# hwwang55/GraphGAN

Measured on AMD Instinct MI355X. Metric: sampled_edges_per_sec, higher is better.
Workload: dtype f32

## Files before the change

### graphgan_amd/csrc/steps.hip

```cpp
#include <stdlib.h>

#include <algorithm>
#include <cmath>
#include <vector>

#include "gg_internal.h"

namespace gg {

struct HubAcc {
    unsigned long long *acc;
    int64_t cap;
    float scale;
};
__device__ __forceinline__ unsigned long long *hub_row(const HubAcc &h, int slot, int ld) {
    const int64_t k = -3 - (int64_t)slot;
    return (slot <= -3 && k < h.cap) ? h.acc + k * (ld + 1) : nullptr;
}
__device__ __forceinline__ void hub_add(unsigned long long *p, float x, float scale) {
    atomicAdd(p, (unsigned long long)__float2ll_rn(x * scale));
}

struct StepArgs {
    float *E, *b;
// ... 549 lines not shown
        }
        if (t == 0) {
            float var = a.b[row];
            const float g = a.gb[row];
            if (SGD) {
                var -= a.lr * g;
            } else {
                float m = a.mb[row], v = a.vb[row];
                adam_elem(var, m, v, g, a);
                a.mb[row] = m;
                a.vb[row] = v;
            }
            if (!__builtin_isfinite(var)) *a.bad = 1ull;
            a.b[row] = var;
            a.gb[row] = 0.f;
            a.touched[row] = 0;
            if (a.sg_cnt) a.sg_cnt[row] = 0;
        }
    }
}

constexpr int DET_MAX_PAIRS = 256;
constexpr int DET_THREADS = 1024;
constexpr int DET_GROUPS = DET_THREADS / 16;
constexpr size_t DET_LDS_ROW_BYTES = 144 * 1024;

__device__ __forceinline__ unsigned group16_ballot(bool pred) {
    const uint64_t m = __ballot(pred);
    return (unsigned)(m >> (threadIdx.x & 48)) & 0xffffu;
}

template <int NF, bool ROWS_IN_LDS, int OPT, bool SMALLN>
__global__ __launch_bounds__(DET_THREADS) void pair_grad_det_kernel(const StepArgs a, const OptArgs o) {
    static_assert(OPT == 0 || ROWS_IN_LDS, "the fused update needs every table read in front of the barrier");
    extern __shared__ float det_rows[];
    __shared__ int32_t ids[2 * DET_MAX_PAIRS];
    __shared__ float coef[DET_MAX_PAIRS], coefb[DET_MAX_PAIRS];
    const int t = threadIdx.x & 15, g = threadIdx.x >> 4;
    const int n = a.n, ld = a.ld, nchunk = ld >> 2;
    const float inv_n = a.n_glob ? 1.0f / (float)(*a.n_glob) : a.inv_n;
    const bool stamp = a.prof && blockIdx.x == 0 && (threadIdx.x == 0 || threadIdx.x == DET_THREADS - 64);
    unsigned long long *const pw = a.prof + (threadIdx.x ? 8 : 0);
    if (stamp) pw[0] = wall_clock64();
    for (int s = threadIdx.x; s < 2 * n; s += DET_THREADS) ids[s] = s < n ? a.u[s] : a.v[s - n];
    for (int p = g; p < n; p += DET_GROUPS) {
        const int iu = a.u[p], iv = a.v[p];
        const float xp = a.x[p];
        const float bv = a.b[iv];
        const float4 *ru = (const float4 *)(a.E + (int64_t)iu * ld);
        const float4 *rv = (const float4 *)(a.E + (int64_t)iv * ld);
        float acc = 0.f;
        for (int c = t; c < nchunk; c += 16) {
            const float4 x = ru[c], y = rv[c];
            if (ROWS_IN_LDS) {
                ((float4 *)(det_rows + (size_t)p * ld))[c] = x;
                ((float4 *)(det_rows + (size_t)(n + p) * ld))[c] = y;
            }
            acc = __builtin_fmaf(x.x, y.x, acc);
            acc = __builtin_fmaf(x.y, y.y, acc);
            acc = __builtin_fmaf(x.z, y.z, acc);
            acc = __builtin_fmaf(x.w, y.w, acc);
        }
        acc += __shfl_xor(acc, 8, 64);
        acc += __shfl_xor(acc, 4, 64);
        acc += __shfl_xor(acc, 2, 64);
        acc += __shfl_xor(acc, 1, 64);
        const float sc = acc + bv;
        const float sg = 1.0f / (1.0f + expf(-sc));
        float ds;
        if (a.is_d) {
            ds = sg - xp;
        } else {
            const bool inside = (sg >= 1e-5f) && (sg <= 1.0f);
            ds = inside ? -(xp * inv_n) * (1.0f - sg) : 0.0f;
        }
        if (t == 0) {
            coef[p] = ds;
            coefb[p] = a.is_d ? ds + a.lambda * bv : ds;
        }
    }
    if (stamp) pw[1] = wall_clock64();
    __syncthreads();
    if (stamp) pw[2] = wall_clock64();
    constexpr int NW = SMALLN ? 2 : 2 * DET_MAX_PAIRS / 64;
    constexpr int NFW = (NF + 3) / 4;
    constexpr int CB = 4;
    const int lane = threadIdx.x & 63;
    const int wave = __builtin_amdgcn_readfirstlane((int)(threadIdx.x >> 6));
    int idr[NW];
#pragma unroll
    for (int j = 0; j < NW; ++j) idr[j] = (64 * j + lane < 2 * n) ? ids[64 * j + lane] : -1;
    auto leader_of = [&](const int s, int &r, uint64_t (&m)[NW]) -> bool {
        r = __builtin_amdgcn_readlane(idr[0], s & 63);
#pragma unroll
        for (int j = 1; j < NW; ++j) r = (s >> 6) == j ? __builtin_amdgcn_readlane(idr[j], s & 63) : r;
        bool earlier = false;
#pragma unroll
        for (int j = 0; j < NW; ++j) {
            m[j] = __ballot(idr[j] == r);
            if (64 * j + 63 < s) earlier |= m[j] != 0ull;
            else if (64 * j <= s) earlier |= (m[j] & ((1ull << (s & 63)) - 1ull)) != 0ull;
        }
        return !earlier;
    };
    auto own_row = [&](const int s, const int r, const uint64_t (&m)[NW], const bool PRE, const float (&pm)[NFW], const float (&pv)[NFW], const float (&pb)[3]) {
        float own[NFW], lown[NFW], acc[NFW], accb = 0.f;
#pragma unroll
        for (int i = 0; i < NFW; ++i) {
            const int f = lane + 64 * i;
            own[i] = f < ld ? (ROWS_IN_LDS ? det_rows[(size_t)s * ld + f] : a.E[(int64_t)r * ld + f]) : 0.f;
            lown[i] = a.lambda * own[i];
            acc[i] = 0.f;
        }
#pragma unroll
        for (int j = 0; j < NW; ++j) {
            uint64_t cur = m[j];
            while (cur) {
                int sq[CB];
#pragma unroll
                for (int k = 0; k < CB; ++k) {
                    if (cur) { sq[k] = 64 * j + __builtin_ctzll(cur); cur &= cur - 1ull; }
                    else sq[k] = -1;
                }
                float c[CB], cb[CB], pr[CB][NFW];
#pragma unroll
                for (int k = 0; k < CB; ++k) {
                    const int sk = sq[k] >= 0 ? sq[k] : s;
                    const int p = sk < n ? sk : sk - n;
                    const int ps = sk < n ? n + p : p;
                    c[k] = coef[p];
                    cb[k] = coefb[p];
                    const float *prow = ROWS_IN_LDS ? det_rows + (size_t)ps * ld : a.E + (int64_t)ids[ps] * ld;
#pragma unroll
                    for (int i = 0; i < NFW; ++i) {
                        const int f = lane + 64 * i;
                        pr[k][i] = f < ld ? prow[f] : 0.f;
                    }
                }
#pragma unroll
                for (int k = 0; k < CB; ++k) {
                    if (sq[k] >= 0) {
#pragma unroll
                        for (int i = 0; i < NFW; ++i) acc[i] += c[k] * pr[k][i] + lown[i];
                        if (sq[k] >= n) accb += cb[k];
                    }
                }
            }
        }
        if (OPT == 0) {
            float *gr = a.gE + (int64_t)r * ld;
#pragma unroll
            for (int i = 0; i < NFW; ++i) {
                const int f = lane + 64 * i;
                if (f < ld) gr[f] = acc[i];
            }
            if (lane == 0) {
                a.gb[r] = accb;
                if (a.track) a.touched[r] = 1;
            }
        } else {
            const int64_t ro = (int64_t)r * ld;
#pragma unroll
            for (int i = 0; i < NFW; ++i) {
                const int f = lane + 64 * i;
                if (f < ld) {
                    float var = own[i];
                    if (OPT == 2) {
                        var -= o.lr * acc[i];
                    } else {
                        float m1 = PRE ? pm[i] : o.mE[ro + f], v1 = PRE ? pv[i] : o.vE[ro + f];
                        adam_elem(var, m1, v1, acc[i], o);
                        o.mE[ro + f] = m1;
                        o.vE[ro + f] = v1;
                    }
                    if (!__builtin_isfinite(var)) *o.bad = 1ull;
                    o.E[ro + f] = var;
                }
            }
            if (lane == 0) {
                float var = PRE ? pb[0] : o.b[r];
                if (OPT == 2) {
                    var -= o.lr * accb;
                } else {
                    float m1 = PRE ? pb[1] : o.mb[r], v1 = PRE ? pb[2] : o.vb[r];
                    adam_elem(var, m1, v1, accb, o);
                    o.mb[r] = m1;
                    o.vb[r] = v1;
                }
                if (!__builtin_isfinite(var)) *o.bad = 1ull;
                o.b[r] = var;
            }
        }
    };
    if constexpr (OPT != 0 && SMALLN && NFW <= 2) {
        constexpr int SPW = 2 * 64 / (DET_THREADS / 64);
        constexpr int SPH = SPW / 2;
#pragma clang loop unroll(full)
        for (int h0 = 0; h0 < SPW; h0 += SPH) {
            float pm[SPH][NFW], pv[SPH][NFW], pb[SPH][3];
#pragma clang loop unroll(full)
            for (int k = 0; k < SPH; ++k) {
                const int s = wave + (h0 + k) * (DET_THREADS / 64);
                int r = 0;
                uint64_t m[NW];
#pragma unroll
                for (int i = 0; i < NFW; ++i) { pm[k][i] = 0.f; pv[k][i] = 0.f; }
                pb[k][0] = pb[k][1] = pb[k][2] = 0.f;
                if (s < 2 * n && leader_of(s, r, m)) {
                    const int64_t ro = (int64_t)r * ld;
#pragma unroll
                    for (int i = 0; i < NFW; ++i) {
                        const int f = lane + 64 * i;
                        if (OPT == 1 && f < ld) { pm[k][i] = o.mE[ro + f]; pv[k][i] = o.vE[ro + f]; }
                    }
                    if (lane == 0) {
                        pb[k][0] = o.b[r];
                        if (OPT == 1) { pb[k][1] = o.mb[r]; pb[k][2] = o.vb[r]; }
                    }
                }
            }
#pragma clang loop unroll(full)
            for (int k = 0; k < SPH; ++k) {
                const int s = wave + (h0 + k) * (DET_THREADS / 64);
                int r = 0;
                uint64_t m[NW];
                if (s < 2 * n && leader_of(s, r, m)) own_row(s, r, m, true, pm[k], pv[k], pb[k]);
            }
        }
    } else {
        const float none[NFW] = {}, none3[3] = {};
        for (int s = (int)blockIdx.x * (DET_THREADS / 64) + wave; s < 2 * n; s += (int)gridDim.x * (DET_THREADS / 64)) {
            int r = 0;
            uint64_t m[NW];
            if (leader_of(s, r, m)) own_row(s, r, m, false, none, none, none3);
        }
    }
    if (stamp) pw[3] = wall_clock64();
}

static unsigned det_workgroups(int n) {
    static const int cap = [] { const char *e = getenv("GG_DET_WORKGROUPS"); return e ? std::max(1, atoi(e)) : 8; }();
    return (unsigned)std::min(cap, std::max(1, (2 * n + DET_THREADS / 64 - 1) / (DET_THREADS / 64)));
}

static bool det_lds_granted(int device);
static bool det_rows_fit_lds(const gg_ctx *ctx, const StepArgs &s) {
    return (size_t)2 * s.n * s.ld * sizeof(float) <= DET_LDS_ROW_BYTES && det_lds_granted(ctx->device);
}

template <int NF, int OPT>
static hipError_t launch_pair_grad_det_lds(gg_ctx *ctx, const StepArgs &s, const OptArgs &o) {
    static bool raised_dev[64] = {};
    bool &raised = raised_dev[ctx->device & 63];
    if (!raised) {
        hipError_t e = hipFuncSetAttribute((const void *)pair_grad_det_kernel<NF, true, OPT, true>, hipFuncAttributeMaxDynamicSharedMemorySize, (int)DET_LDS_ROW_BYTES);
        if (e == hipSuccess) e = hipFuncSetAttribute((const void *)pair_grad_det_kernel<NF, true, OPT, false>, hipFuncAttributeMaxDynamicSharedMemorySize, (int)DET_LDS_ROW_BYTES);
        if (e != hipSuccess) return e;
        raised = true;
    }
    const size_t dyn = (size_t)2 * s.n * s.ld * sizeof(float);
    const dim3 grid(OPT == 0 ? det_workgroups(s.n) : 1);
    if (s.n <= 64) hipLaunchKernelGGL((pair_grad_det_kernel<NF, true, OPT, true>), grid, dim3(DET_THREADS), dyn, ctx->stream, s, o);
    else hipLaunchKernelGGL((pair_grad_det_kernel<NF, true, OPT, false>), grid, dim3(DET_THREADS), dyn, ctx->stream, s, o);
    return hipSuccess;
}

static bool det_lds_granted(int device) {
    static int state[64] = {};
    int &s = state[device & 63];
    if (s == 0) {
        const hipError_t e = hipFuncSetAttribute((const void *)pair_grad_det_kernel<4, true, 0, true>, hipFuncAttributeMaxDynamicSharedMemorySize, (int)DET_LDS_ROW_BYTES);
        if (e != hipSuccess) (void)hipGetLastError();
        s = e == hipSuccess ? 1 : -1;
    }
    return s > 0;
}

template <int NF>
static hipError_t launch_pair_grad_det(gg_ctx *ctx, const StepArgs &s, const OptArgs &o, int opt) {
    if (!det_rows_fit_lds(ctx, s)) {
        const dim3 grid(det_workgroups(s.n));
        if (s.n <= 64) hipLaunchKernelGGL((pair_grad_det_kernel<NF, false, 0, true>), grid, dim3(DET_THREADS), 0, ctx->stream, s, o);
        else hipLaunchKernelGGL((pair_grad_det_kernel<NF, false, 0, false>), grid, dim3(DET_THREADS), 0, ctx->stream, s, o);
        return hipSuccess;
    }
    if (opt == 1) return launch_pair_grad_det_lds<NF, 1>(ctx, s, o);
    if (opt == 2) return launch_pair_grad_det_lds<NF, 2>(ctx, s, o);
    return launch_pair_grad_det_lds<NF, 0>(ctx, s, o);
}

template <int SGD>
__global__ __launch_bounds__(256) void sparse_opt_kernel(const OptArgs a) {
    const int t = threadIdx.x & 15;
    const int g0 = (blockIdx.x * blockDim.x + threadIdx.x) >> 4;
    const int ng = (gridDim.x * blockDim.x) >> 4;
    const int cnt = (int)*a.touched_total;
    const int nchunk = a.ld >> 2;
    for (int r = g0; r < cnt; r += ng) opt_row<SGD>(a, a.touched_list[r], t, nchunk);
}

constexpr int STAGE_SORT = 64;

template <int MODE>
__global__ __launch_bounds__(256) void staged_opt_kernel(const OptArgs a) {
    constexpr bool SGD = MODE == 1;
    __shared__ int32_t perm_s[16][STAGE_SORT];
    const int t = threadIdx.x & 15;
    int32_t *const perm = perm_s[threadIdx.x >> 4];
    const int64_t g0 = ((int64_t)blockIdx.x * blockDim.x + threadIdx.x) >> 4, ng = ((int64_t)gridDim.x * blockDim.x) >> 4;
    const int64_t n_rows = a.sg_tot[0];
    const int nchunk = a.ld >> 2;
    for (int64_t r = g0; r < n_rows; r += ng) {
        const int4 e = a.sg_list[r];
        const int row = e.x, n = e.z;
        const float4 *const seg = (const float4 *)(a.stage + (int64_t)e.y * a.ld);
        const float *const sb = a.stage_b + e.y;
        const int32_t *const key = a.stage_key + e.y;
        float4 g[4];
#pragma unroll
        for (int i = 0; i < 4; ++i) g[i] = make_float4(0.f, 0.f, 0.f, 0.f);
        float gbias = 0.f;
        auto add_row = [&](const float4 *src) {
#pragma unroll
            for (int i = 0; i < 4; ++i) {
                const int c = t + 16 * i;
                if (c < nchunk) {
                    const float4 x = src[c];
                    g[i].x += x.x; g[i].y += x.y; g[i].z += x.z; g[i].w += x.w;
                }
            }
        };
        if (n <= STAGE_SORT) {
            if (n > 1) {
                int k[4], rk[4];
#pragma unroll
                for (int i = 0; i < 4; ++i) {
                    k[i] = (t + 16 * i < n) ? key[t + 16 * i] : 0x7fffffff;
                    rk[i] = 0;
                }
#pragma unroll
                for (int j = 0; j < 4; ++j) {
                    if (16 * j < n) {
                        const int nl = min(n - 16 * j, 16);
                        for (int l = 0; l < nl; ++l) {
                            const int kk = __shfl(k[j], l, 16);
#pragma unroll
                            for (int i = 0; i < 4; ++i) rk[i] += kk < k[i];
                        }
                    }
                }
#pragma unroll
                for (int i = 0; i < 4; ++i)
                    if (t + 16 * i < n) perm[rk[i]] = t + 16 * i;
            } else if (t == 0) {
                perm[0] = 0;
            }
            __builtin_amdgcn_fence(__ATOMIC_RELEASE, "wavefront");
            __builtin_amdgcn_wave_barrier();
            __builtin_amdgcn_fence(__ATOMIC_ACQUIRE, "wavefront");
            int o = 0;
            for (; o + 4 <= n; o += 4) {
                const float4 *s0 = seg + (int64_t)perm[o] * nchunk, *s1 = seg + (int64_t)perm[o + 1] * nchunk;
                const float4 *s2 = seg + (int64_t)perm[o + 2] * nchunk, *s3 = seg + (int64_t)perm[o + 3] * nchunk;
#pragma unroll
                for (int i = 0; i < 4; ++i) {
                    const int c = t + 16 * i;
                    if (c < nchunk) {
                        const float4 x0 = s0[c], x1 = s1[c], x2 = s2[c], x3 = s3[c];
                        g[i].x += x0.x; g[i].y += x0.y; g[i].z += x0.z; g[i].w += x0.w;
                        g[i].x += x1.x; g[i].y += x1.y; g[i].z += x1.z; g[i].w += x1.w;
                        g[i].x += x2.x; g[i].y += x2.y; g[i].z += x2.z; g[i].w += x2.w;
                        g[i].x += x3.x; g[i].y += x3.y; g[i].z += x3.z; g[i].w += x3.w;
                    }
                }
            }
            for (; o < n; ++o) add_row(seg + (int64_t)perm[o] * nchunk);
            for (int q = t; q < n; q += 16) gbias += sb[perm[q]];
            __builtin_amdgcn_wave_barrier();
        } else {
            int last = -1;
            for (int q = 0; q < n; ++q) {
                int best = 0x7fffffff, besto = 0;
                for (int o = t; o < n; o += 16) {
                    const int kk = key[o];
                    if (kk > last && kk < best) { best = kk; besto = o; }
                }
#pragma unroll
                for (int m = 8; m >= 1; m >>= 1) {
                    const int ob = __shfl_xor(best, m, 16), oo = __shfl_xor(besto, m, 16);
                    if (ob < best) { best = ob; besto = oo; }
                }
                add_row(seg + (int64_t)besto * nchunk);
                if ((q & 15) == t) gbias += sb[besto];
                last = best;
            }
        }
        gbias += __shfl_xor(gbias, 8, 64);
        gbias += __shfl_xor(gbias, 4, 64);
        gbias += __shfl_xor(gbias, 2, 64);
        gbias += __shfl_xor(gbias, 1, 64);
        const int64_t o4 = ((int64_t)row * a.ld) >> 2;
        if (MODE == 2) {
#pragma unroll
            for (int i = 0; i < 4; ++i) {
                const int c = t + 16 * i;
                if (c < nchunk) ((float4 *)a.gE)[o4 + c] = g[i];
            }
            if (t == 0) {
                a.gb[row] = gbias;
                a.touched[row] = 1;
                a.sg_cnt[row] = 0;
            }
            continue;
        }
#pragma unroll
        for (int i = 0; i < 4; ++i) {
            const int c = t + 16 * i;
            if (c >= nchunk) continue;
            float4 var = ((float4 *)a.E)[o4 + c];
            if (SGD) {
                var.x -= a.lr * g[i].x; var.y -= a.lr * g[i].y; var.z -= a.lr * g[i].z; var.w -= a.lr * g[i].w;
            } else {
                float4 m = ((float4 *)a.mE)[o4 + c], v = ((float4 *)a.vE)[o4 + c];
                adam_elem(var.x, m.x, v.x, g[i].x, a);
                adam_elem(var.y, m.y, v.y, g[i].y, a);
                adam_elem(var.z, m.z, v.z, g[i].z, a);
                adam_elem(var.w, m.w, v.w, g[i].w, a);
                ((float4 *)a.mE)[o4 + c] = m;
                ((float4 *)a.vE)[o4 + c] = v;
            }
            if (nonfinite4(var)) *a.bad = 1ull;
            ((float4 *)a.E)[o4 + c] = var;
        }
        if (t == 0) {
            float var = a.b[row];
            if (SGD) {
                var -= a.lr * gbias;
            } else {
                float m = a.mb[row], v = a.vb[row];
                adam_elem(var, m, v, gbias, a);
                a.mb[row] = m;
                a.vb[row] = v;
            }
            if (!__builtin_isfinite(var)) *a.bad = 1ull;
            a.b[row] = var;
            a.sg_cnt[row] = 0;
        }
    }
}

__global__ void add_word_kernel(int64_t *dst, const int64_t *src) { *dst += *src; }

__global__ __launch_bounds__(256) void pack_rows_kernel(float *gE, float *gb, int32_t *touched, const int32_t *list, const int64_t *cnt_ptr,
                                                        int64_t cap, int ld, int32_t *out_ids, float *out_rows, int32_t *err) {
    const int t = threadIdx.x & 15;
    const int64_t g0 = ((int64_t)blockIdx.x * blockDim.x + threadIdx.x) >> 4, ng = ((int64_t)gridDim.x * blockDim.x) >> 4;
    const int64_t cnt = *cnt_ptr;
    if (cnt > cap && blockIdx.x == 0 && threadIdx.x == 0) *err = 1;
    for (int64_t r = g0; r < cap; r += ng) {
        if (r >= cnt) {
            if (t == 0) out_ids[r] = -1;
            continue;
        }
        const int row = list[r];
        float *src = gE + (int64_t)row * ld, *dst = out_rows + r * (ld + 1);
        for (int f = t; f < ld; f += 16) { dst[f] = src[f]; src[f] = 0.f; }
        if (t == 0) { dst[ld] = gb[row]; gb[row] = 0.f; out_ids[r] = row; touched[row] = 0; }
    }
}

__device__ __forceinline__ uint16_t f32_to_bf16(float x) {
    uint32_t u = __builtin_bit_cast(uint32_t, x);
    if ((u & 0x7fffffffu) > 0x7f800000u) return (uint16_t)((u >> 16) | 0x40u);
    u += 0x7fffu + ((u >> 16) & 1u);
    return (uint16_t)(u >> 16);
}
__device__ __forceinline__ float bf16_to_f32(uint16_t h) { return __builtin_bit_cast(float, (uint32_t)h << 16); }
static inline size_t pack_row_words(int ld, bool bf16) { return bf16 ? (size_t)(ld + 2) / 2 : (size_t)ld + 1; }
template <bool BF16> __device__ __forceinline__ float pack_get(const float *rows, int64_t r, int ld, int f) {
    if (BF16) return bf16_to_f32(((const uint16_t *)rows)[r * (ld + 2) + f]);
    return rows[r * (ld + 1) + f];
}
template <bool BF16> __device__ __forceinline__ void pack_put(float *rows, int64_t r, int ld, int f, float v) {
    if (BF16) ((uint16_t *)rows)[r * (ld + 2) + f] = f32_to_bf16(v);
    else rows[r * (ld + 1) + f] = v;
}

template <bool BF16 = false>
__global__ __launch_bounds__(256) void add_rows_kernel(float *gE, float *gb, int32_t *touched, const int32_t *ids, const float *rows, int64_t cnt,
                                                       int ld) {
    const int t = threadIdx.x & 15;
    const int64_t g0 = ((int64_t)blockIdx.x * blockDim.x + threadIdx.x) >> 4, ng = ((int64_t)gridDim.x * blockDim.x) >> 4;
    for (int64_t r = g0; r < cnt; r += ng) {
        const int row = ids[r];
        if (row < 0) continue;
        float *dst = gE + (int64_t)row * ld;
        for (int f = t; f < ld; f += 16) dst[f] += pack_get<BF16>(rows, r, ld, f);
        if (t == 0) { gb[row] += pack_get<BF16>(rows, r, ld, ld); touched[row] = 1; }
    }
}


int apply_optimizer(gg_ctx *ctx, int which, int64_t n);
void step_done(gg_ctx *ctx, int which, int64_t n);
int run_path_step(gg_ctx *ctx);

static OptArgs make_opt_args(gg_ctx *ctx, int which) {
    Model &M = ctx->model[which];
    OptArgs o{};
    o.E = M.E; o.b = M.b; o.mE = M.mE; o.vE = M.vE; o.mb = M.mb; o.vb = M.vb; o.gE = ctx->gradE; o.gb = ctx->gradb;
    o.nE = (int64_t)ctx->n_node * ctx->ld;
    o.n_node = ctx->n_node; o.ld = ctx->ld;
    o.b1 = ctx->cfg.adam_beta1; o.b2 = ctx->cfg.adam_beta2; o.eps = ctx->cfg.adam_eps;
    o.lr = M.lr;
    o.lr_t = (M.lr * sqrtf(1.0f - M.b2p)) / (1.0f - M.b1p);
    o.touched = ctx->touched; o.touched_list = ctx->touched_list; o.touched_cnt = ctx->touched_cnt;
    o.bad = ctx->table_bad.as<unsigned long long>() + which;
    return o;
}

__global__ void set_count_kernel(int64_t *dst, int64_t v) { *dst = v; }

static int global_pair_count(gg_ctx *ctx, int64_t n_local, const int64_t **out) {
    *out = nullptr;
    const int world = ctx->comm ? ctx->world : ctx->fake_world;
    if (world <= 1) return GG_OK;
    GG_HIP(ctx, ctx->x_nglob.reserve(sizeof(int64_t) * 2));
    int64_t *w = ctx->x_nglob.as<int64_t>();
    hipLaunchKernelGGL(set_count_kernel, dim3(1), dim3(1), 0, ctx->stream, w, ctx->comm ? n_local : n_local * world);
    if (ctx->comm) {
        int rc = comm_allreduce_i64(ctx, w, 1);
        if (rc != GG_OK) return rc;
    }
    *out = w;
    return GG_OK;
}

static int64_t stage_bytes_cap() {
    static const int64_t cap = [] {
        const char *e = getenv("GG_STAGE_MAX_BYTES");
        return e ? (int64_t)atoll(e) : (int64_t)24 << 30;
    }();
    return cap;
}

__global__ __launch_bounds__(256) void hub_index_kernel(const int32_t *cnt, int64_t n, int T, int32_t *off, int32_t *rows, int64_t *nhub) {
    const int64_t i = (int64_t)blockIdx.x * blockDim.x + threadIdx.x;
    if (i >= n || cnt[i] <= T) return;
    const int h = (int)atomicAdd((unsigned long long *)nhub, 1ull);
    off[i] = h;
    rows[h] = (int32_t)i;
}

__global__ __launch_bounds__(256) void hub_finalize_kernel(unsigned long long *acc, const int32_t *rows, const int64_t *nhub, int64_t cap, int ld,
                                                           double inv_scale, float *gE, float *gb) {
    const int64_t n = min(*nhub, cap) * (ld + 1);
    for (int64_t i = (int64_t)blockIdx.x * blockDim.x + threadIdx.x; i < n; i += (int64_t)gridDim.x * blockDim.x) {
        const unsigned long long v = acc[i];
        if (!v) continue;
        acc[i] = 0ull;
        const int64_t h = i / (ld + 1);
        const int f = (int)(i - h * (ld + 1));
        const float x = (float)((double)(long long)v * inv_scale);
        if (f < ld) gE[(int64_t)rows[h] * ld + f] += x;
        else gb[rows[h]] += x;
    }
}

static float hub_scale(bool per_pair_mean, int64_t n) {
    return std::ldexp(1.0f, 32 + (per_pair_mean && n > 1 ? (int)std::ilogb((double)n) : 0));
}

static HubAcc hub_args(gg_ctx *ctx, float scale) {
    return HubAcc{ctx->hub_acc.as<unsigned long long>(), ctx->hub_cap, scale};
}

static int hub_index(gg_ctx *ctx, const int32_t *cnt, int32_t *off, DevBuf &rows, int64_t *tot, hipStream_t stream) {
    GG_HIP(ctx, rows.reserve(sizeof(int32_t) * (size_t)ctx->n_node));
    GG_HIP(ctx, hipMemsetAsync(tot + 2, 0, sizeof(int64_t), stream));
    hipLaunchKernelGGL(hub_index_kernel, dim3((unsigned)cdiv(ctx->n_node, 256)), dim3(256), 0, stream, cnt, (int64_t)ctx->n_node, ctx->sg_threshold, off,
                       rows.as<int32_t>(), tot + 2);
    GG_HIP(ctx, hipGetLastError());
    return GG_OK;
}

static void hub_finalize(gg_ctx *ctx, bool early_index, float scale, float *gE, float *gb) {
    DevBuf &rows = early_index ? ctx->sgp_hub : ctx->sg_hub, &tot = early_index ? ctx->sgp_tot : ctx->sg_tot;
    const int64_t n = ctx->hub_cap * (ctx->ld + 1);
    const unsigned nb = (unsigned)std::max<int64_t>(1, std::min<int64_t>(cdiv(n, 256), 2048));
    hipLaunchKernelGGL(hub_finalize_kernel, dim3(nb), dim3(256), 0, ctx->stream, ctx->hub_acc.as<unsigned long long>(), rows.as<int32_t>(),
                       tot.as<int64_t>() + 2, ctx->hub_cap, ctx->ld, 1.0 / (double)scale, gE, gb);
}

static int staged_reserve(gg_ctx *ctx, int64_t n_occ, int64_t n_stage) {
    if (n_stage * (int64_t)(ctx->ld + 2) * 4 > stage_bytes_cap()) return 1;
    const size_t cnt_before = ctx->sg_cnt.bytes;
    GG_HIP(ctx, ctx->sg_cnt.reserve(sizeof(int32_t) * (size_t)ctx->n_node));
    const bool was_dirty = ctx->sg_cnt_dirty;
    if (ctx->sg_cnt.bytes != cnt_before || ctx->sg_cnt_dirty) GG_HIP(ctx, hipMemsetAsync(ctx->sg_cnt.p, 0, ctx->sg_cnt.bytes, ctx->stream));
    ctx->sg_cnt_dirty = true;
    GG_HIP(ctx, ctx->sg_off.reserve(sizeof(int32_t) * (size_t)ctx->n_node));
    GG_HIP(ctx, ctx->sg_list.reserve(sizeof(int4) * (size_t)ctx->n_node));
    GG_HIP(ctx, ctx->sg_slot.reserve(sizeof(int32_t) * (size_t)n_occ));
    GG_HIP(ctx, ctx->sg_bias.reserve(sizeof(float) * (size_t)n_stage));
    GG_HIP(ctx, ctx->sg_key.reserve(sizeof(int32_t) * (size_t)n_stage));
    GG_HIP(ctx, ctx->sg_tot.reserve(sizeof(int64_t) * 4));
    {
        const int64_t cap = std::min<int64_t>(ctx->n_node, n_occ / ((int64_t)ctx->sg_threshold + 1) + 1);
        const size_t before = ctx->hub_acc.bytes;
        if (ctx->hub_acc.reserve(sizeof(unsigned long long) * (size_t)cap * (ctx->ld + 1)) != hipSuccess) {
            (void)hipGetLastError();
            ctx->hub_cap = 0;
            return 1;
        }
        if (ctx->hub_acc.bytes != before || was_dirty) GG_HIP(ctx, hipMemsetAsync(ctx->hub_acc.p, 0, ctx->hub_acc.bytes, ctx->stream));
        ctx->hub_cap = (int64_t)(ctx->hub_acc.bytes / (sizeof(unsigned long long) * (ctx->ld + 1)));
    }
    if (ctx->sg_rows.reserve(sizeof(float) * (size_t)n_stage * ctx->ld) != hipSuccess) {
        (void)hipGetLastError();
        return 1;
    }
    return GG_OK;
}

static int staged_finish(gg_ctx *ctx, int which, int64_t n, int64_t n_occ, bool early_index = false) {
    const int opt = ctx->cfg.optimizer;
    OptArgs o = make_opt_args(ctx, which);
    DevBuf &b_cnt = early_index ? ctx->sgp_cnt : ctx->sg_cnt, &b_list = early_index ? ctx->sgp_list : ctx->sg_list;
    DevBuf &b_tot = early_index ? ctx->sgp_tot : ctx->sg_tot, &b_key = early_index ? ctx->sgp_key : ctx->sg_key;
    o.sg_cnt = b_cnt.as<int32_t>(); o.sg_list = b_list.as<int4>(); o.sg_tot = b_tot.as<int64_t>();
    o.stage = ctx->sg_rows.as<float>(); o.stage_b = ctx->sg_bias.as<float>(); o.stage_key = b_key.as<int32_t>();
    int nb = cdiv((int64_t)std::min<int64_t>(n_occ, ctx->n_node) * 16, 256);
    if (nb > 4096) nb = 4096;
    if (nb < 1) nb = 1;
    const bool replicas = ctx->comm || ctx->fake_world > 1;
    if (replicas) hipLaunchKernelGGL(staged_opt_kernel<2>, dim3(nb), dim3(256), 0, ctx->stream, o);
    else if (opt == GG_OPT_SGD) hipLaunchKernelGGL(staged_opt_kernel<1>, dim3(nb), dim3(256), 0, ctx->stream, o);
    else hipLaunchKernelGGL(staged_opt_kernel<0>, dim3(nb), dim3(256), 0, ctx->stream, o);
    ctx->sg_active = true;
    ctx->sg_cnt_active = o.sg_cnt;
    const int rc = apply_optimizer(ctx, which, n);
    ctx->sg_active = false;
    if (rc != GG_OK) return rc;
    if (!replicas)
        hipLaunchKernelGGL(add_word_kernel, dim3(1), dim3(1), 0, ctx->stream, ctx->touched_ptr.as<int64_t>() + ctx->n_node, b_tot.as<int64_t>());
    GG_HIP(ctx, hipGetLastError());
    if (early_index) ctx->sgp_cnt_clean = true;
    else ctx->sg_cnt_dirty = false;
    return GG_OK;
}

static bool staged_allowed(const gg_ctx *ctx) {
    return ctx->sg_threshold > 0 && ctx->ld <= 256 && ctx->cfg.optimizer != GG_OPT_ADAM_DENSE && !getenv("GG_NO_STAGED_GRAD");
}

int run_step(gg_ctx *ctx, int which, const int32_t *d_u, const int32_t *d_v, const float *d_x, int32_t n) {
    if (n <= 0) return GG_OK;
    Model &M = ctx->model[which];
    const int opt = ctx->cfg.optimizer;
    StepArgs s{};
    s.E = M.E; s.b = M.b; s.gE = ctx->gradE; s.gb = ctx->gradb;
    s.touched = ctx->touched; s.touched_list = ctx->touched_list; s.touched_cnt = ctx->touched_cnt;
    s.ld = ctx->ld;
    s.track = opt != GG_OPT_ADAM_DENSE;
    s.u = d_u; s.v = d_v; s.x = d_x; s.n = n;
    s.lambda = M.lambda;
    s.inv_n = 1.0f / (float)n;
    s.is_d = which == 1;
    if (which == 0) {
        int rc = global_pair_count(ctx, n, &s.n_glob);
        if (rc != GG_OK) return rc;
    }
    s.ppg = n >= 16384 ? PAIRS_PER_GROUP : (n >= 2048 ? 4 : 1);
    if (ctx->deterministic && n <= DET_MAX_PAIRS) {
        const int nfd = (ctx->ld + 15) / 16;
        const bool replicas = ctx->comm || ctx->fake_world > 1;
        const int fused = (!replicas && opt != GG_OPT_ADAM_DENSE && det_rows_fit_lds(ctx, s) && !getenv("GG_NO_FUSED_SMALL_STEP")) ? (opt == GG_OPT_SGD ? 2 : 1) : 0;
        const OptArgs o = make_opt_args(ctx, which);
        static unsigned long long *det_prof = nullptr;
        static const bool det_prof_on = getenv("GG_DET_PROFILE") != nullptr;
        if (det_prof_on) {
            if (!det_prof) GG_HIP(ctx, hipMalloc((void **)&det_prof, 16 * sizeof(unsigned long long)));
            GG_HIP(ctx, hipMemsetAsync(det_prof, 0, 16 * sizeof(unsigned long long), ctx->stream));
            s.prof = det_prof;
        }
        hipError_t e;
        if (nfd <= 4) e = launch_pair_grad_det<4>(ctx, s, o, fused);
        else if (nfd <= 8) e = launch_pair_grad_det<8>(ctx, s, o, fused);
        else if (nfd <= 16) e = launch_pair_grad_det<16>(ctx, s, o, fused);
        else e = launch_pair_grad_det<32>(ctx, s, o, fused);
        GG_HIP(ctx, e);
        if (det_prof_on) {
            static double acc_t[2][2][4] = {};
            static long cnt[2] = {};
            unsigned long long h[16];
            GG_HIP(ctx, hipMemcpyAsync(h, det_prof, sizeof(h), hipMemcpyDeviceToHost, ctx->stream));
            GG_HIP(ctx, hipStreamSynchronize(ctx->stream));
            for (int w = 0; w < 2; ++w)
                for (int k = 0; k < 3; ++k) acc_t[which][w][k] += h[8 * w + k + 1] > h[8 * w + k] ? 10.0 * (double)(h[8 * w + k + 1] - h[8 * w + k]) : 0.0;
            if (++cnt[which] % 1000 == 0)
                for (int w = 0; w < 2; ++w)
                    fprintf(stderr, "[det] model %d n=%d wave %s: loads+coef %.0f ns, barrier %.0f, owners' sums + stores issued %.0f (means over %ld steps)\n", which, n, w ? "15" : "0",
                            acc_t[which][w][0] / cnt[which], acc_t[which][w][1] / cnt[which], acc_t[which][w][2] / cnt[which], cnt[which]);
        }
        if (fused) {
            GG_HIP(ctx, hipGetLastError());
            step_done(ctx, which, n);
            return GG_OK;
        }
        return apply_optimizer(ctx, which, n);
    }
    const int groups = cdiv(n, s.ppg);
    const int blocks = cdiv((int64_t)groups * 16, 256);
    const int nf = (ctx->ld + 15) / 16;
    bool staged = n >= 16384 && n < (1 << 30) && staged_allowed(ctx);
    if (staged) {
        int rc = staged_reserve(ctx, 2 * (int64_t)n, 2 * (int64_t)n);
        if (rc < 0) return rc;
        if (rc == 1) staged = false;
    }
    if (staged) {
        int rc;
        int32_t *cnt = ctx->sg_cnt.as<int32_t>(), *off = ctx->sg_off.as<int32_t>(), *slot_v = ctx->sg_slot.as<int32_t>(), *slot_u = slot_v + n;
        hipLaunchKernelGGL(pair_occ_count_kernel, dim3(cdiv(n, 256)), dim3(256), 0, ctx->stream, d_u, d_v, n, s.ppg, cnt, slot_v, slot_u);
        rc = device_segment_rows(ctx, cnt, ctx->n_node, ctx->sg_threshold, off, ctx->sg_list.as<int4>(), ctx->sg_tot.as<int64_t>());
        if (rc != GG_OK) return rc;
        rc = hub_index(ctx, cnt, off, ctx->sg_hub, ctx->sg_tot.as<int64_t>(), ctx->stream);
        if (rc != GG_OK) return rc;
        hipLaunchKernelGGL(pair_occ_slot_kernel, dim3(cdiv(n, 256)), dim3(256), 0, ctx->stream, d_u, d_v, n, cnt, off, ctx->sg_threshold, slot_v, slot_u,
                           ctx->sg_key.as<int32_t>());
        s.slot_v = slot_v; s.slot_u = slot_u;
        s.stage = ctx->sg_rows.as<float>(); s.stage_b = ctx->sg_bias.as<float>();
        const float scale = hub_scale(!s.is_d, n);
        s.hub = hub_args(ctx, scale);
        if (nf <= 4) hipLaunchKernelGGL((pair_grad16_kernel<4, true>), dim3(blocks), dim3(256), 0, ctx->stream, s);
        else if (nf <= 8) hipLaunchKernelGGL((pair_grad16_kernel<8, true>), dim3(blocks), dim3(256), 0, ctx->stream, s);
        else hipLaunchKernelGGL((pair_grad16_kernel<16, true>), dim3(blocks), dim3(256), 0, ctx->stream, s);
        hub_finalize(ctx, false, scale, s.gE, s.gb);
        if (ctx->tm_cur >= 0) GG_HIP(ctx, hipEventRecord(ctx->tm_ev[ctx->tm_cur][1], ctx->stream));
        return staged_finish(ctx, which, n, 2 * (int64_t)n);
    }
    if (s.ppg == PAIRS_PER_GROUP && nf <= 16 && !getenv("GG_OLD_PAIR_GRAD")) {
        if (nf <= 4) hipLaunchKernelGGL((pair_grad16_kernel<4, false>), dim3(blocks), dim3(256), 0, ctx->stream, s);
        else if (nf <= 8) hipLaunchKernelGGL((pair_grad16_kernel<8, false>), dim3(blocks), dim3(256), 0, ctx->stream, s);
        else hipLaunchKernelGGL((pair_grad16_kernel<16, false>), dim3(blocks), dim3(256), 0, ctx->stream, s);
    } else if (nf <= 4) hipLaunchKernelGGL((pair_grad_kernel<4, false>), dim3(blocks), dim3(256), 0, ctx->stream, s);
    else if (nf <= 8) hipLaunchKernelGGL((pair_grad_kernel<8, false>), dim3(blocks), dim3(256), 0, ctx->stream, s);
    else if (nf <= 16) hipLaunchKernelGGL((pair_grad_kernel<16, false>), dim3(blocks), dim3(256), 0, ctx->stream, s);
    else hipLaunchKernelGGL((pair_grad_kernel<32, false>), dim3(blocks), dim3(256), 0, ctx->stream, s);
    if (ctx->tm_cur >= 0) GG_HIP(ctx, hipEventRecord(ctx->tm_ev[ctx->tm_cur][1], ctx->stream));

    return apply_optimizer(ctx, which, n);
}

template <bool STAGED>
static void launch_path_grad(gg_ctx *ctx, const PathArgs &p, int blocks, int nf) {
    const dim3 g(blocks), b(256);
    if (p.stride <= 17) {
        if (nf <= 4) hipLaunchKernelGGL((path_grad_kernel<4, STAGED, true>), g, b, 0, ctx->stream, p);
        else if (nf <= 8) hipLaunchKernelGGL((path_grad_kernel<8, STAGED, true>), g, b, 0, ctx->stream, p);
        else hipLaunchKernelGGL((path_grad_kernel<16, STAGED, true>), g, b, 0, ctx->stream, p);
    } else {
        if (nf <= 4) hipLaunchKernelGGL((path_grad_kernel<4, STAGED, false>), g, b, 0, ctx->stream, p);
        else if (nf <= 8) hipLaunchKernelGGL((path_grad_kernel<8, STAGED, false>), g, b, 0, ctx->stream, p);
        else hipLaunchKernelGGL((path_grad_kernel<16, STAGED, false>), g, b, 0, ctx->stream, p);
    }
}

int run_path_step(gg_ctx *ctx) {
    Model &M = ctx->model[0];
    const int64_t n = ctx->g_pairs;
    PathArgs p{};
    p.E = M.E; p.b = M.b; p.gE = ctx->gradE; p.gb = ctx->gradb;
    p.touched = ctx->touched; p.touched_list = ctx->touched_list; p.touched_cnt = ctx->touched_cnt;
    p.ld = ctx->ld;
    p.track = ctx->cfg.optimizer != GG_OPT_ADAM_DENSE;
    p.window = ctx->cfg.window_size;
    p.paths = ctx->w_paths.as<int32_t>();
    p.path_len = ctx->w_len.as<int32_t>();
    p.stride = ctx->w_stride;
    p.pair_ptr = ctx->g_ptr.as<int64_t>();
    p.reward = ctx->g_reward.as<float>();
    p.n_walks = ctx->w_total;
    p.lambda = M.lambda;
    p.inv_n = 1.0f / (float)n;
    {
        int rc = global_pair_count(ctx, n, &p.n_glob);
        if (rc != GG_OK) return rc;
    }
    const int blocks = cdiv(p.n_walks * 16, 256);
    const int nf = (ctx->ld + 15) / 16;
    const int64_t n_pos = p.n_walks * (int64_t)p.stride;
    bool staged = staged_allowed(ctx) && n_pos < (1ll << 31);
    const int64_t n_stage = std::min<int64_t>(n_pos, p.window >= 2 ? (n + 6 * p.n_walks) / 4 + 1 : (n + 2 * p.n_walks) / 2 + 1);
    if (staged) {
        const int rc = staged_reserve(ctx, n_pos, n_stage);
        if (rc < 0) return rc;
        if (rc == 1) staged = false;
    }
    if (!staged) {
        launch_path_grad<false>(ctx, p, blocks, nf);
        if (ctx->tm_cur >= 0) GG_HIP(ctx, hipEventRecord(ctx->tm_ev[ctx->tm_cur][1], ctx->stream));
        return apply_optimizer(ctx, 0, n);
    }
    int rc;
    int32_t *cnt = ctx->sg_cnt.as<int32_t>(), *off = ctx->sg_off.as<int32_t>(), *slot = ctx->sg_slot.as<int32_t>();
    const dim3 pgrid((unsigned)cdiv(n_pos, 256));
    const bool early = ctx->g_slots_ready && ctx->g_slots_walks == p.n_walks && ctx->g_slots_stride == p.stride;
    ctx->g_slots_ready = false;
    ctx->g_slots_unused = 0;
    if (early) {
        ctx->sg_cnt_dirty = false;
        GG_HIP(ctx, hipStreamWaitEvent(ctx->stream, ctx->ev_slots_done, 0));
        slot = ctx->sgp_slot.as<int32_t>();
    } else {
        hipLaunchKernelGGL(path_count_kernel, pgrid, dim3(256), 0, ctx->stream, p.paths, p.path_len, p.stride, p.n_walks, cnt, slot, (const unsigned long long *)nullptr);
        rc = device_segment_rows(ctx, cnt, ctx->n_node, ctx->sg_threshold, off, ctx->sg_list.as<int4>(), ctx->sg_tot.as<int64_t>());
        if (rc != GG_OK) return rc;
        rc = hub_index(ctx, cnt, off, ctx->sg_hub, ctx->sg_tot.as<int64_t>(), ctx->stream);
        if (rc != GG_OK) return rc;
        hipLaunchKernelGGL(path_slot_kernel, pgrid, dim3(256), 0, ctx->stream, p.paths, p.path_len, p.stride, p.n_walks, cnt, off, ctx->sg_threshold, slot,
                           ctx->sg_key.as<int32_t>(), (const unsigned long long *)nullptr);
    }
    p.slot = slot;
    p.stage = ctx->sg_rows.as<float>();
    p.stage_b = ctx->sg_bias.as<float>();
    const float scale = hub_scale(true, n);
    p.hub = hub_args(ctx, scale);
    launch_path_grad<true>(ctx, p, blocks, nf);
    hub_finalize(ctx, early, scale, p.gE, p.gb);
    if (ctx->tm_cur >= 0) GG_HIP(ctx, hipEventRecord(ctx->tm_ev[ctx->tm_cur][1], ctx->stream));
    return staged_finish(ctx, 0, n, n_pos, early);
}

int enqueue_path_slots(gg_ctx *ctx) {
    ctx->g_slots_ready = false;
    if (ctx->walk_stream == ctx->stream || ctx->in_epoch_add || getenv("GG_NO_EARLY_SLOTS")) return GG_OK;
    const int64_t n_walks = ctx->w_total, n_pos = n_walks * (int64_t)ctx->w_stride;
    if (!staged_allowed(ctx) || ctx->cfg.window_size > 2 || n_walks == 0 || n_pos >= (1ll << 31)) return GG_OK;
    if (ctx->g_slots_unused >= 2) {
        if (ctx->sgp_slot.p) {
            for (DevBuf *b : {&ctx->sgp_cnt, &ctx->sgp_off, &ctx->sgp_slot, &ctx->sgp_list, &ctx->sgp_key, &ctx->sgp_scan, &ctx->sgp_hub}) b->release();
            ctx->sgp_cnt_clean = false;
        }
        return GG_OK;
    }
    hipStream_t st = ctx->walk_stream;
    const size_t cnt_before = ctx->sgp_cnt.bytes;
    GG_HIP(ctx, ctx->sgp_cnt.reserve(sizeof(int32_t) * (size_t)ctx->n_node));
    if (ctx->sgp_cnt.bytes != cnt_before || !ctx->sgp_cnt_clean) GG_HIP(ctx, hipMemsetAsync(ctx->sgp_cnt.p, 0, ctx->sgp_cnt.bytes, st));
    ctx->sgp_cnt_clean = false;
    GG_HIP(ctx, ctx->sgp_off.reserve(sizeof(int32_t) * (size_t)ctx->n_node));
    GG_HIP(ctx, ctx->sgp_list.reserve(sizeof(int4) * (size_t)ctx->n_node));
    GG_HIP(ctx, ctx->sgp_slot.reserve(sizeof(int32_t) * (size_t)n_pos));
    GG_HIP(ctx, ctx->sgp_key.reserve(sizeof(int32_t) * (size_t)n_pos));
    GG_HIP(ctx, ctx->sgp_tot.reserve(sizeof(int64_t) * 4));
    if (!ctx->ev_slots_done) GG_HIP(ctx, hipEventCreateWithFlags(&ctx->ev_slots_done, hipEventDisableTiming));
    const unsigned long long *flag = ctx->dev_ctr + 3;
    const dim3 pgrid((unsigned)cdiv(n_pos, 256));
    int32_t *cnt = ctx->sgp_cnt.as<int32_t>(), *off = ctx->sgp_off.as<int32_t>(), *slot = ctx->sgp_slot.as<int32_t>();
    hipLaunchKernelGGL(path_count_kernel, pgrid, dim3(256), 0, st, ctx->w_paths.as<int32_t>(), ctx->w_len.as<int32_t>(), ctx->w_stride, n_walks, cnt, slot, flag);
    int rc = device_segment_rows(ctx, cnt, ctx->n_node, ctx->sg_threshold, off, ctx->sgp_list.as<int4>(), ctx->sgp_tot.as<int64_t>(), st, &ctx->sgp_scan);
    if (rc != GG_OK) return rc;
    rc = hub_index(ctx, cnt, off, ctx->sgp_hub, ctx->sgp_tot.as<int64_t>(), st);
    if (rc != GG_OK) return rc;
    hipLaunchKernelGGL(path_slot_kernel, pgrid, dim3(256), 0, st, ctx->w_paths.as<int32_t>(), ctx->w_len.as<int32_t>(), ctx->w_stride, n_walks, cnt, off,
                       ctx->sg_threshold, slot, ctx->sgp_key.as<int32_t>(), flag);
    GG_HIP(ctx, hipGetLastError());
    GG_HIP(ctx, hipEventRecord(ctx->ev_slots_done, st));
    ctx->g_slots_ready = true;
    ctx->g_slots_walks = n_walks;
    ctx->g_slots_stride = ctx->w_stride;
    return GG_OK;
}

__global__ void normalize_flags_kernel(int32_t *f, int n) {
    const int i = blockIdx.x * blockDim.x + threadIdx.x;
    if (i < n && f[i] > 1) f[i] = 1;
}

__global__ void scale_grads_kernel(float *gE, float *gb, int64_t nE, int n, float k) {
    const int64_t stride = (int64_t)gridDim.x * blockDim.x;
    for (int64_t i = (int64_t)blockIdx.x * blockDim.x + threadIdx.x; i < nE; i += stride) gE[i] *= k;
    for (int64_t i = (int64_t)blockIdx.x * blockDim.x + threadIdx.x; i < n; i += stride) gb[i] *= k;
}

__global__ __launch_bounds__(256) void owner_count_kernel(const int32_t *list, const int64_t *cnt_ptr, int world, long long *cnt) {
    __shared__ int sh[64];
    if (threadIdx.x < 64) sh[threadIdx.x] = 0;
    __syncthreads();
    const int64_t n = *cnt_ptr;
    for (int64_t i = (int64_t)blockIdx.x * blockDim.x + threadIdx.x; i < n; i += (int64_t)gridDim.x * blockDim.x) atomicAdd(&sh[list[i] % world], 1);
    __syncthreads();
    if ((int)threadIdx.x < world && sh[threadIdx.x]) atomicAdd((unsigned long long *)&cnt[threadIdx.x], (unsigned long long)sh[threadIdx.x]);
}

template <bool BF16>
__global__ __launch_bounds__(256) void owner_pack_kernel(const float *gE, const float *gb, const int32_t *list, const int64_t *cnt_ptr, int world,
                                                         const long long *seg_off, long long *fill, int ld, int32_t *out_ids, float *out_rows) {
    const int t = threadIdx.x & 15;
    const int64_t g0 = ((int64_t)blockIdx.x * blockDim.x + threadIdx.x) >> 4, ng = ((int64_t)gridDim.x * blockDim.x) >> 4;
    const int64_t cnt = *cnt_ptr;
    for (int64_t r = g0; r < cnt; r += ng) {
        const int row = list[r];
        const int q = row % world;
        long long slot = 0;
        if (t == 0) slot = seg_off[q] + (long long)atomicAdd((unsigned long long *)&fill[q], 1ull);
        slot = __shfl(slot, (threadIdx.x & 63) & ~15, 64);
        const float *src = gE + (int64_t)row * ld;
        for (int f = t; f < ld; f += 16) pack_put<BF16>(out_rows, slot, ld, f, src[f]);
        if (t == 0) {
            pack_put<BF16>(out_rows, slot, ld, ld, gb[row]);
            if (BF16) pack_put<BF16>(out_rows, slot, ld, ld + 1, 0.f);
            out_ids[slot] = row;
        }
    }
}

template <bool BF16>
__global__ __launch_bounds__(256) void owner_gather_pack_kernel(float *gE, float *gb, const int32_t *list, const int64_t *cnt_ptr, int world,
                                                                int me, long long *fill, int64_t cap, int ld, int32_t *out_ids, float *out_rows) {
    const int t = threadIdx.x & 15;
    const int64_t g0 = ((int64_t)blockIdx.x * blockDim.x + threadIdx.x) >> 4, ng = ((int64_t)gridDim.x * blockDim.x) >> 4;
    const int64_t cnt = *cnt_ptr;
    for (int64_t r = g0; r < cnt; r += ng) {
        const int row = list[r];
        if (row % world != me) continue;
        long long slot = 0;
        if (t == 0) slot = (long long)atomicAdd((unsigned long long *)fill, 1ull);
        slot = __shfl(slot, (threadIdx.x & 63) & ~15, 64);
        if (slot >= cap) continue;
        float *src = gE + (int64_t)row * ld;
        for (int f = t; f < ld; f += 16) {
            pack_put<BF16>(out_rows, slot, ld, f, src[f]);
            if (BF16) src[f] = pack_get<BF16>(out_rows, slot, ld, f);
        }
        if (t == 0) {
            pack_put<BF16>(out_rows, slot, ld, ld, gb[row]);
            if (BF16) { gb[row] = pack_get<BF16>(out_rows, slot, ld, ld); pack_put<BF16>(out_rows, slot, ld, ld + 1, 0.f); }
            out_ids[slot] = row;
        }
// ... 413 lines not shown
```

Measured before the change: 637.4 million.

## Rewrite staged optimizer kernel with prefetching, DPP rank sort and ld-specialized chunks

Replaces the staged gradient-apply optimizer kernel with a new version that prefetches the next list entries and keys one or two iterations ahead and loads parameter and optimizer state before reducing staged rows. For segments of up to 16 rows it computes sort ranks in registers with DPP row rotations and ds_permute instead of going through shared memory, and it unrolls the row accumulation four rows at a time. A template parameter specializes the chunk count for ld==128. The old kernel stays available behind an environment variable. The cost is more register pressure and more code complexity.

```diff
diff --git a/graphgan_amd/csrc/steps.hip b/graphgan_amd/csrc/steps.hip
--- a/graphgan_amd/csrc/steps.hip
+++ b/graphgan_amd/csrc/steps.hip
@@ -875,7 +875,7 @@
 constexpr int STAGE_SORT = 64;
 
 template <int MODE>
-__global__ __launch_bounds__(256) void staged_opt_kernel(const OptArgs a) {
+__global__ __launch_bounds__(256) void staged_opt_old_kernel(const OptArgs a) {
     constexpr bool SGD = MODE == 1;
     __shared__ int32_t perm_s[16][STAGE_SORT];
     const int t = threadIdx.x & 15;
@@ -1020,6 +1020,210 @@
             a.sg_cnt[row] = 0;
         }
     }
+}
+
+template <int S> __device__ __forceinline__ int row_ror(int x) { return __builtin_amdgcn_update_dpp(0, x, 0x120 + S, 0xf, 0xf, false); }
+template <int S = 1> __device__ __forceinline__ int rank16(int k) {
+    if constexpr (S == 16) return 0;
+    else return (row_ror<S>(k) < k ? 1 : 0) + rank16<S + 1>(k);
+}
+
+template <int MODE, int NC>
+__global__ __launch_bounds__(256) void staged_opt_kernel(const OptArgs a) {
+    constexpr bool SGD = MODE == 1;
+    __shared__ int32_t perm_s[16][STAGE_SORT];
+    const int t = threadIdx.x & 15;
+    const int lane0 = threadIdx.x & 48;
+    int32_t *const perm = perm_s[threadIdx.x >> 4];
+    const int64_t g0 = ((int64_t)blockIdx.x * blockDim.x + threadIdx.x) >> 4, ng = ((int64_t)gridDim.x * blockDim.x) >> 4;
+    const int64_t n_rows = a.sg_tot[0];
+    if (g0 >= n_rows) return;
+    const int nchunk = a.ld >> 2;
+    int cc[NC];
+#pragma unroll
+    for (int i = 0; i < NC; ++i) cc[i] = NC == 2 ? t + 16 * i : min(t + 16 * i, nchunk - 1);
+    auto has = [&](int i) { return NC == 2 || t + 16 * i < nchunk; };
+    auto fetch_keys = [&](const int4 &x, int (&k)[4]) {
+        const int32_t *const key = a.stage_key + x.y;
+#pragma unroll
+        for (int i = 0; i < 4; ++i) {
+            const int kk = key[min(t + 16 * i, x.z - 1)];
+            k[i] = t + 16 * i < x.z ? kk : 0x7fffffff;
+        }
+    };
+    auto entry = [&](int64_t r) { return a.sg_list[min(r, n_rows - 1)]; };
+    int4 e = entry(g0), en = entry(g0 + ng);
+    int k[4], kn[4];
+    fetch_keys(e, k);
+    for (int64_t r = g0; r < n_rows; r += ng) {
+        const int row = e.x, n = e.z;
+        const float4 *const seg = (const float4 *)(a.stage + (int64_t)e.y * a.ld);
+        const float *const sb = a.stage_b + e.y;
+        const int64_t o4 = ((int64_t)row * a.ld) >> 2;
+        float4 var[NC], mm[NC], vv[NC];
+        float bvar = 0.f, bm = 0.f, bv = 0.f;
+        if (MODE != 2) {
+#pragma unroll
+            for (int i = 0; i < NC; ++i) {
+                var[i] = ((const float4 *)a.E)[o4 + cc[i]];
+                if (!SGD) {
+                    mm[i] = ((const float4 *)a.mE)[o4 + cc[i]];
+                    vv[i] = ((const float4 *)a.vE)[o4 + cc[i]];
+                }
+            }
+            bvar = a.b[row];
+            if (!SGD) { bm = a.mb[row]; bv = a.vb[row]; }
+        }
+        fetch_keys(en, kn);
+        const int4 enn = entry(r + 2 * ng);
+        float4 g[NC];
+#pragma unroll
+        for (int i = 0; i < NC; ++i) g[i] = make_float4(0.f, 0.f, 0.f, 0.f);
+        float gbias = 0.f;
+        auto add_row = [&](const float4 *src) {
+#pragma unroll
+            for (int i = 0; i < NC; ++i) {
+                const float4 x = src[cc[i]];
+                if (has(i)) { g[i].x += x.x; g[i].y += x.y; g[i].z += x.z; g[i].w += x.w; }
+            }
+        };
+        if (n <= 16) {
+            int p = 0;
+            if (n > 1) {
+                const int rk = rank16(k[0]);
+                p = __builtin_amdgcn_ds_permute((lane0 + (t < n ? rk : t)) << 2, t);
+            }
+            int o = 0;
+            for (; o + 4 <= n; o += 4) {
+                const float4 *s0 = seg + (int64_t)__shfl(p, o, 16) * nchunk, *s1 = seg + (int64_t)__shfl(p, o + 1, 16) * nchunk;
+                const float4 *s2 = seg + (int64_t)__shfl(p, o + 2, 16) * nchunk, *s3 = seg + (int64_t)__shfl(p, o + 3, 16) * nchunk;
+#pragma unroll
+                for (int i = 0; i < NC; ++i) {
+                    const float4 x0 = s0[cc[i]], x1 = s1[cc[i]], x2 = s2[cc[i]], x3 = s3[cc[i]];
+                    if (has(i)) {
+                        g[i].x += x0.x; g[i].y += x0.y; g[i].z += x0.z; g[i].w += x0.w;
+                        g[i].x += x1.x; g[i].y += x1.y; g[i].z += x1.z; g[i].w += x1.w;
+                        g[i].x += x2.x; g[i].y += x2.y; g[i].z += x2.z; g[i].w += x2.w;
+                        g[i].x += x3.x; g[i].y += x3.y; g[i].z += x3.z; g[i].w += x3.w;
+                    }
+                }
+            }
+            for (; o < n; ++o) add_row(seg + (int64_t)__shfl(p, o, 16) * nchunk);
+            const float bq = sb[t < n ? p : 0];
+            if (t < n) gbias += bq;
+        } else if (n <= STAGE_SORT) {
+            int rk[4] = {0, 0, 0, 0};
+#pragma unroll
+            for (int j = 0; j < 4; ++j) {
+                if (16 * j < n) {
+                    const int nl = min(n - 16 * j, 16);
+                    for (int l = 0; l < nl; ++l) {
+                        const int kk = __shfl(k[j], l, 16);
+#pragma unroll
+                        for (int i = 0; i < 4; ++i) rk[i] += kk < k[i];
+                    }
+                }
+            }
+#pragma unroll
+            for (int i = 0; i < 4; ++i)
+                if (t + 16 * i < n) perm[rk[i]] = t + 16 * i;
+            __builtin_amdgcn_fence(__ATOMIC_RELEASE, "wavefront");
+            __builtin_amdgcn_wave_barrier();
+            __builtin_amdgcn_fence(__ATOMIC_ACQUIRE, "wavefront");
+            int o = 0;
+            for (; o + 4 <= n; o += 4) {
+                const float4 *s0 = seg + (int64_t)perm[o] * nchunk, *s1 = seg + (int64_t)perm[o + 1] * nchunk;
+                const float4 *s2 = seg + (int64_t)perm[o + 2] * nchunk, *s3 = seg + (int64_t)perm[o + 3] * nchunk;
+#pragma unroll
+                for (int i = 0; i < NC; ++i) {
+                    const float4 x0 = s0[cc[i]], x1 = s1[cc[i]], x2 = s2[cc[i]], x3 = s3[cc[i]];
+                    if (has(i)) {
+                        g[i].x += x0.x; g[i].y += x0.y; g[i].z += x0.z; g[i].w += x0.w;
+                        g[i].x += x1.x; g[i].y += x1.y; g[i].z += x1.z; g[i].w += x1.w;
+                        g[i].x += x2.x; g[i].y += x2.y; g[i].z += x2.z; g[i].w += x2.w;
+                        g[i].x += x3.x; g[i].y += x3.y; g[i].z += x3.z; g[i].w += x3.w;
+                    }
+                }
+            }
+            for (; o < n; ++o) add_row(seg + (int64_t)perm[o] * nchunk);
+            for (int q = t; q < n; q += 16) gbias += sb[perm[q]];
+            __builtin_amdgcn_wave_barrier();
+        } else {
+            const int32_t *const key = a.stage_key + e.y;
+            int last = -1;
+            for (int q = 0; q < n; ++q) {
+                int best = 0x7fffffff, besto = 0;
+                for (int o = t; o < n; o += 16) {
+                    const int kk = key[o];
+                    if (kk > last && kk < best) { best = kk; besto = o; }
+                }
+#pragma unroll
+                for (int m = 8; m >= 1; m >>= 1) {
+                    const int ob = __shfl_xor(best, m, 16), oo = __shfl_xor(besto, m, 16);
+                    if (ob < best) { best = ob; besto = oo; }
+                }
+                add_row(seg + (int64_t)besto * nchunk);
+                if ((q & 15) == t) gbias += sb[besto];
+                last = best;
+            }
+        }
+        e = en;
+        en = enn;
+#pragma unroll
+        for (int i = 0; i < 4; ++i) k[i] = kn[i];
+        gbias += __shfl_xor(gbias, 8, 64);
+        gbias += __shfl_xor(gbias, 4, 64);
+        gbias += __shfl_xor(gbias, 2, 64);
+        gbias += __shfl_xor(gbias, 1, 64);
+        if (MODE == 2) {
+#pragma unroll
+            for (int i = 0; i < NC; ++i)
+                if (has(i)) ((float4 *)a.gE)[o4 + cc[i]] = g[i];
+            if (t == 0) {
+                a.gb[row] = gbias;
+                a.touched[row] = 1;
+                a.sg_cnt[row] = 0;
+            }
+            continue;
+        }
+#pragma unroll
+        for (int i = 0; i < NC; ++i) {
+            if (!has(i)) continue;
+            float4 x = var[i];
+            if (SGD) {
+                x.x -= a.lr * g[i].x; x.y -= a.lr * g[i].y; x.z -= a.lr * g[i].z; x.w -= a.lr * g[i].w;
+            } else {
+                adam_elem(x.x, mm[i].x, vv[i].x, g[i].x, a);
+                adam_elem(x.y, mm[i].y, vv[i].y, g[i].y, a);
+                adam_elem(x.z, mm[i].z, vv[i].z, g[i].z, a);
+                adam_elem(x.w, mm[i].w, vv[i].w, g[i].w, a);
+                ((float4 *)a.mE)[o4 + cc[i]] = mm[i];
+                ((float4 *)a.vE)[o4 + cc[i]] = vv[i];
+            }
+            if (nonfinite4(x)) *a.bad = 1ull;
+            ((float4 *)a.E)[o4 + cc[i]] = x;
+        }
+        if (t == 0) {
+            float x = bvar;
+            if (SGD) {
+                x -= a.lr * gbias;
+            } else {
+                adam_elem(x, bm, bv, gbias, a);
+                a.mb[row] = bm;
+                a.vb[row] = bv;
+            }
+            if (!__builtin_isfinite(x)) *a.bad = 1ull;
+            a.b[row] = x;
+            a.sg_cnt[row] = 0;
+        }
+    }
+}
+
+template <int MODE>
+static void launch_staged_opt(gg_ctx *ctx, int nb, const OptArgs &o) {
+    if (getenv("GG_OLD_STAGED_OPT")) hipLaunchKernelGGL(staged_opt_old_kernel<MODE>, dim3(nb), dim3(256), 0, ctx->stream, o);
+    else if (ctx->ld == 128) hipLaunchKernelGGL((staged_opt_kernel<MODE, 2>), dim3(nb), dim3(256), 0, ctx->stream, o);
+    else hipLaunchKernelGGL((staged_opt_kernel<MODE, 4>), dim3(nb), dim3(256), 0, ctx->stream, o);
 }
 
 __global__ void add_word_kernel(int64_t *dst, const int64_t *src) { *dst += *src; }
@@ -1207,9 +1411,9 @@
     if (nb > 4096) nb = 4096;
     if (nb < 1) nb = 1;
     const bool replicas = ctx->comm || ctx->fake_world > 1;
-    if (replicas) hipLaunchKernelGGL(staged_opt_kernel<2>, dim3(nb), dim3(256), 0, ctx->stream, o);
-    else if (opt == GG_OPT_SGD) hipLaunchKernelGGL(staged_opt_kernel<1>, dim3(nb), dim3(256), 0, ctx->stream, o);
-    else hipLaunchKernelGGL(staged_opt_kernel<0>, dim3(nb), dim3(256), 0, ctx->stream, o);
+    if (replicas) launch_staged_opt<2>(ctx, nb, o);
+    else if (opt == GG_OPT_SGD) launch_staged_opt<1>(ctx, nb, o);
+    else launch_staged_opt<0>(ctx, nb, o);
     ctx->sg_active = true;
     ctx->sg_cnt_active = o.sg_cnt;
     const int rc = apply_optimizer(ctx, which, n);
```

Result: no change. 645.4 million (median of 6 runs) (+1.2%).
